# zihuixue/DynMM

Measured on AMD Instinct MI355X. Metric: images/sec fwd+bwd, 480x640 RGB-D, batch 32/GPU, higher is better.
Workload: dtype f32; 1 GPU; configs[2]: zero-grad + fwd + weighted 4-scale CE + FLOP loss + bwd + fused SGD-Nesterov update, --dynamic --global-gate soft DiffSoftmax gates tau=1; per_gpu_batch=32, global_batch=32, height=480, width=640, parallelism=dp1, launch=eager, streams=4, optimizer_in_step=fused SGD-Nesterov

## Files before the change

### dynmm_amd/csrc/conv_wino.hip

```cpp
#include <stdlib.h>

#include "common.h"
#include "conv_igemm.h"

namespace dynmm {

struct WinoArgs {
    const float* x;
    const float* ut;
    const float* shift;
    const float* residual;
    const float* mask;
    float* y;
    double* stats;
    const float *bn_mean, *bn_invstd, *bn_gamma, *bn_beta;
    const unsigned long long* bits;
    int nslots;
    int N, Ci, Co, H, W;
    int CoS;
    int act;
    int MP;
    int H2;
    int n_co_tiles, n_p_tiles;
    int Hin, Win;
};

__device__ __forceinline__ float quad_sum(float v) {
    v += __int_as_float(__builtin_amdgcn_mov_dpp(__float_as_int(v), 0xB1, 0xF, 0xF, true));
    v += __int_as_float(__builtin_amdgcn_mov_dpp(__float_as_int(v), 0x4E, 0xF, 0xF, true));
    return v;
}

template <int TCO, int MCO, bool VERT, bool DGRAD, bool S2 = false, bool TAIL = false, bool STATS = false, int BNRED = 0>
__global__ void __launch_bounds__(256, MCO == 1 ? ((VERT && !DGRAD) ? 4 : 3) : 2) conv_wino_kernel(const WinoArgs a) {
    static_assert(!BNRED || (DGRAD && VERT && !S2 && MCO == 1 && TCO == 64 && !TAIL && !STATS), "BatchNorm reductions: vertical dgrad");
    static_assert(!S2 || DGRAD, "the stride-2 form is an input gradient");
    static_assert(!STATS || (!DGRAD && !VERT && MCO == 1 && TCO == 64 && !TAIL), "statistics: the forward's small horizontal tile");
    static_assert(!TAIL || (!DGRAD && MCO == 1), "channel tails exist in the forward's small tile only");
    constexpr int S = (VERT && !DGRAD && MCO == 1) ? 2 : 3;
    constexpr int BK = 8;
    constexpr int WCO = 32 * MCO;
    constexpr int WAVES_CO = TCO / WCO, WAVES_P = 4 / WAVES_CO, TP = 32 * WAVES_P;
    static_assert(WAVES_CO * WAVES_P == 4 && (MCO == 1 || MCO == 2), "4 waves per workgroup");
    constexpr int A_STAGE = BK * TCO * 4;
    constexpr int PIXW = (S2 ? TP : 2 * TP) + 8;
    constexpr int NP = S2 ? 2 : 4;
    constexpr int B_STAGE = VERT ? BK * NP * TP : BK * PIXW;
    constexpr int QPR = VERT ? TP / 4 : PIXW / 4;
    constexpr int QB = B_STAGE / 4, QPW = QB / 4;
    constexpr int NIB = (QPW + 63) / 64;
    constexpr int IPR = TCO / 64;
    constexpr int NIA = 2 * IPR;
    constexpr int NI = NIA + NIB;
    static_assert(NI < 64 && QB % 4 == 0, "vmcnt is a 6-bit counter; the four waves split a stage evenly");

    __shared__ __attribute__((aligned(16))) float As[S * A_STAGE];
    __shared__ __attribute__((aligned(16))) float Bs[S * B_STAGE];

    const int t = threadIdx.x;
    const int lane = t & 63;
    const int wave = __builtin_amdgcn_readfirstlane(t >> 6);
    const int wave_co = wave / WAVES_P, wave_p = wave % WAVES_P;
    const int khalf = lane >> 5, l31 = lane & 31;

    const int nblk = a.n_co_tiles * a.n_p_tiles;
    const int lin = xcd_remap((int)blockIdx.x, nblk);
    const int co0 = (lin % a.n_co_tiles) * TCO;
    const int p0 = (lin / a.n_co_tiles) * TP;
    const int HW = a.H * a.W;
    const int HWin = a.Hin * a.Win;
    const int NC = a.Ci / BK;
    const int nst = NC;

    unsigned b_off[NIB];
    bool b_act[NIB];
#pragma unroll
    for (int i = 0; i < NIB; ++i) {
        const int ql = i * 64 + lane;
        b_act[i] = ql < QPW;
        const int q = wave * QPW + (b_act[i] ? ql : 0);
        if constexpr (VERT) {
            const int k = q / (NP * QPR), j = (q / QPR) % NP, gq = q % QPR;
            int p = p0 + 4 * gq;
            p = p > a.MP - 4 ? a.MP - 4 : p;
            const int per = a.H2 * a.W;
            const int n = p / per, rr = p - n * per;
            const int r2 = rr / a.W, w = rr - r2 * a.W;
            const int row = S2 ? r2 + j : 2 * r2 - 1 + j;
            const int rowc = (row >= 0 && row < a.Hin) ? row : (S2 ? r2 : 2 * r2);
            b_off[i] = ((unsigned)(n * a.Ci + k) * (unsigned)HWin + (unsigned)(rowc * a.Win + w)) * 4u;
        } else {
            const int k = q / QPR, quad = q - k * QPR;
            const int M = S2 ? a.MP : 2 * a.MP;
            int m = (S2 ? p0 : 2 * p0) - 4 + 4 * quad;
            m = m < 0 ? 0 : (m > M - 4 ? M - 4 : m);
            const int n = m / HWin, rem = m - n * HWin;
            b_off[i] = ((unsigned)(n * a.Ci + k) * (unsigned)HWin + (unsigned)rem) * 4u;
        }
    }
    const unsigned a_voff = (unsigned)lane * 16u;
    const unsigned lds_a = (unsigned)reinterpret_cast<uintptr_t>((__attribute__((address_space(3))) float*)As);
    const unsigned lds_b = (unsigned)reinterpret_cast<uintptr_t>((__attribute__((address_space(3))) float*)Bs);
    const float* a_ptr = a.ut + ((size_t)(2 * wave) * a.CoS + co0) * 4;
    const size_t a_step = (size_t)BK * a.CoS * 4, a_row = (size_t)a.CoS * 4;
    const float* b_ptr = a.x;
    const size_t b_step = (size_t)BK * HWin;
    unsigned l_adst = lds_a + (unsigned)(2 * wave * TCO * 4 * 4), l_bdst = lds_b + (unsigned)(wave * QPW * 4 * 4);
    const unsigned l_adst_end = l_adst + (unsigned)(S * A_STAGE * 4);
    int l_left = nst;
    auto issue = [&]() {
        if (l_left > 0) {
#pragma unroll
            for (int i = 0; i < NIA; ++i)
                dma16(a_ptr + (size_t)(i / IPR) * a_row + 64 * (i % IPR) * 4, a_voff, l_adst + (unsigned)i * 1024u);
#pragma unroll
            for (int i = 0; i < NIB; ++i) {
                if (b_act[i]) dma16(b_ptr, b_off[i], l_bdst + (unsigned)i * 1024u);
            }
            --l_left;
            a_ptr += a_step;
            b_ptr += b_step;
            l_adst += (unsigned)(A_STAGE * 4);
            l_bdst += (unsigned)(B_STAGE * 4);
            if (l_adst == l_adst_end) {
                l_adst -= (unsigned)(S * A_STAGE * 4);
                l_bdst -= (unsigned)(S * B_STAGE * 4);
            }
        }
    };

    const int lp = wave_p * 32 + l31;
    const int p = p0 + lp;
    const bool pvalid = p < a.MP;
    int pn, prem;
    bool m0, m2, m3;
    {
        const int pc = pvalid ? p : 0;
        if constexpr (VERT) {
            const int per = a.H2 * a.W;
            pn = pc / per;
            const int rr = pc - pn * per;
            const int r2 = rr / a.W, w = rr - r2 * a.W;
            prem = 2 * r2 * a.W + w;
            m0 = r2 > 0;
            m2 = 2 * r2 + 1 < a.H;
            m3 = S2 ? r2 + 1 < a.Hin : 2 * r2 + 2 < a.H;
        } else {
            const int m = 2 * pc;
            pn = m / HW;
            prem = m - pn * HW;
            const int h = prem / a.W, w = prem - h * a.W;
            m0 = w > 0;
            m2 = true;
            m3 = S2 ? (w >> 1) + 1 < a.Win : w + 2 < a.W;
        }
    }
    const int a_frag = (khalf * TCO + wave_co * WCO + l31) * 4;
    const int b_frag = VERT ? khalf * NP * TP + lp : (S2 ? khalf * PIXW + 4 + lp : khalf * PIXW + 2 * lp + 2);

    f32x16 acc[4][MCO];
#pragma unroll
    for (int i = 0; i < 4; ++i)
#pragma unroll
        for (int mi = 0; mi < MCO; ++mi)
#pragma unroll
            for (int j = 0; j < 16; ++j) acc[i][mi][j] = 0.f;

    float4 fa[2][MCO];
    float fd[2][4];
    float fv[2][4];
    auto read_raw = [&](int set, int q, const float* Ap, const float* Bp) {
#pragma unroll
        for (int mi = 0; mi < MCO; ++mi)
            fa[set][mi] = *reinterpret_cast<const float4*>(Ap + a_frag + (2 * q * TCO + mi * 32) * 4);
        if constexpr (S2) {
            const float* b = Bp + b_frag + 2 * q * (VERT ? NP * TP : PIXW);
            fd[set][0] = b[0];
            fd[set][1] = b[VERT ? TP : 1];
            fd[set][2] = fd[set][3] = 0.f;
        } else if constexpr (VERT) {
            const float* b = Bp + b_frag + 2 * q * 4 * TP;
            fd[set][0] = b[0];
            fd[set][1] = b[TP];
            fd[set][2] = b[2 * TP];
            fd[set][3] = b[3 * TP];
        } else {
            const float* b = Bp + b_frag + 2 * q * PIXW;
            const float2 u1 = *reinterpret_cast<const float2*>(b + 2);
            fd[set][0] = b[1];
            fd[set][1] = u1.x;
            fd[set][2] = u1.y;
            fd[set][3] = b[4];
        }
    };
    auto transform = [&](int set) {
        if constexpr (S2) {
            fv[set][0] = fv[set][1] = fd[set][0];
            fv[set][2] = m3 ? fd[set][1] : 0.f;
            fv[set][3] = 0.f;
            return;
        }
        const float d0 = m0 ? fd[set][0] : 0.f, d1 = fd[set][1];
        const float d2 = (VERT && !m2) ? 0.f : fd[set][2], d3 = m3 ? fd[set][3] : 0.f;
        fv[set][0] = d0 - d2;
        fv[set][1] = d1 + d2;
        fv[set][2] = d2 - d1;
        fv[set][3] = d1 - d3;
    };
    auto mfma_set = [&](int set) {
#pragma unroll
        for (int mi = 0; mi < MCO; ++mi) {
            const float av[4] = {fa[set][mi].x, fa[set][mi].y, fa[set][mi].z, fa[set][mi].w};
            if constexpr (S2) {
                acc[0][mi] = __builtin_amdgcn_mfma_f32_32x32x2f32(av[0], fv[set][0], acc[0][mi], 0, 0, 0);
                acc[1][mi] = __builtin_amdgcn_mfma_f32_32x32x2f32(av[1], fv[set][1], acc[1][mi], 0, 0, 0);
                acc[1][mi] = __builtin_amdgcn_mfma_f32_32x32x2f32(av[2], fv[set][2], acc[1][mi], 0, 0, 0);
                continue;
            }
#pragma unroll
            for (int i = 0; i < 4; ++i)
                acc[i][mi] = __builtin_amdgcn_mfma_f32_32x32x2f32(av[i], fv[set][i], acc[i][mi], 0, 0, 0);
        }
    };
#define DYNMM_WINO_PHASE() __builtin_amdgcn_sched_barrier(0)

    static_assert(BK == 8, "four k-pairs per stage");
#pragma unroll
    for (int i = 0; i < S; ++i) issue();
    wait_vm<(S - 1) * NI>();
    __syncthreads();
    int c_a = 0, c_b = 0;
    const float* Ap = As;
    const float* Bp = Bs;
    read_raw(0, 0, Ap, Bp);
    transform(0);
    for (int s = 0; s < nst; ++s) {
        DYNMM_WINO_PHASE();
        read_raw(1, 1, Ap, Bp);
        DYNMM_WINO_PHASE();
        mfma_set(0);
        DYNMM_WINO_PHASE();
        transform(1);
        DYNMM_WINO_PHASE();
        read_raw(0, 2, Ap, Bp);
        DYNMM_WINO_PHASE();
        mfma_set(1);
        DYNMM_WINO_PHASE();
        transform(0);
        DYNMM_WINO_PHASE();
        read_raw(1, 3, Ap, Bp);
        DYNMM_WINO_PHASE();
        mfma_set(0);
        DYNMM_WINO_PHASE();
        transform(1);
        DYNMM_WINO_PHASE();
        if (s + 1 < nst) {
            if (S > 2 && s + 2 < nst) wait_vm<(S - 2) * NI>();
            else wait_vm<0>();
            __syncthreads();
            issue();
            c_a += A_STAGE;
            c_b += B_STAGE;
            if (c_a == S * A_STAGE) { c_a = 0; c_b = 0; }
            Ap = As + c_a;
            Bp = Bs + c_b;
            read_raw(0, 0, Ap, Bp);
        }
        DYNMM_WINO_PHASE();
        mfma_set(1);
        DYNMM_WINO_PHASE();
        transform(0);
    }
#undef DYNMM_WINO_PHASE
    const float* __restrict__ res_p = a.residual;
    const float* __restrict__ mask_p = a.mask;
    float* __restrict__ y_p = a.y;
    const bool has_res = res_p != nullptr, has_mask = mask_p != nullptr;
    const int act = a.act;
    const unsigned row_bytes = (unsigned)HW * 4u;
    const unsigned second = VERT ? (unsigned)a.W * 4u : 4u;
    const bool y1_ok = VERT ? m2 : true;
    const unsigned off_base = ((unsigned)(pn * a.Co + co0 + wave_co * WCO + 4 * khalf) * (unsigned)HW + (unsigned)prem) * 4u;
    auto off_of = [&](int b, int e) {
        return off_base + (unsigned)((b >> 1) * 32 + (e & 3) + 8 * (2 * (b & 1) + (e >> 2))) * row_bytes;
    };
    const int co_lim = a.Co - (co0 + wave_co * WCO + 4 * khalf);
    auto live = [&](int b, int e) { return !TAIL || (b >> 1) * 32 + (e & 3) + 8 * (2 * (b & 1) + (e >> 2)) < co_lim; };
    constexpr int NSET = BNRED == 2 ? 1 : 2;
    float k0[NSET][8], k1[NSET][8], r0[NSET][8], r1[NSET][8];
    unsigned w0[NSET][8], w1[NSET][8];
    const unsigned bit_groups = (unsigned)((HW + 255) >> 8);
    auto bit_byte = [&](int i) { return (unsigned)(((i >> 8) * 4 + (i & 3)) * 8 + ((((i & 255) >> 2) >> 5) * 4)); };
    const unsigned bit_off0 = bit_byte(prem), bit_off1 = bit_byte(prem + a.W);
    const unsigned bit_sh0 = (unsigned)(((prem & 255) >> 2) & 31), bit_sh1 = (unsigned)((((prem + a.W) & 255) >> 2) & 31);
    const unsigned bit_plane0 = (unsigned)(pn * a.Co + co0 + wave_co * WCO + 4 * khalf) * bit_groups * 32u;
#pragma unroll
    for (int e = 0; e < 8; ++e)
#pragma unroll
        for (int q = 0; q < NSET; ++q) {
            r0[q][e] = r1[q][e] = 0.f;
            k0[q][e] = k1[q][e] = 1.f;
        }
    auto load_batch = [&](int set, int b) {
#pragma unroll
        for (int e = 0; e < 8; ++e) {
            const unsigned off = off_of(b, e);
            r0[set][e] = r1[set][e] = 0.f;
            k0[set][e] = k1[set][e] = 1.f;
            if constexpr (BNRED == 2) w0[set][e] = w1[set][e] = 0u;
            if (!pvalid || !live(b, e)) continue;
            if constexpr (BNRED == 2) {
                const char* wp_ = reinterpret_cast<const char*>(a.bits) + bit_plane0 +
                                  (unsigned)((b >> 1) * 32 + (e & 3) + 8 * (2 * (b & 1) + (e >> 2))) * bit_groups * 32u;
                w0[set][e] = *reinterpret_cast<const unsigned*>(wp_ + bit_off0);
                w1[set][e] = y1_ok ? *reinterpret_cast<const unsigned*>(wp_ + bit_off1) : 0u;
            }
            if constexpr (VERT) {
                if (has_mask) {
                    k0[set][e] = *reinterpret_cast<const float*>(reinterpret_cast<const char*>(mask_p) + off);
                    if (y1_ok) k1[set][e] = *reinterpret_cast<const float*>(reinterpret_cast<const char*>(mask_p) + off + second);
                }
                if (has_res) {
                    r0[set][e] = *reinterpret_cast<const float*>(reinterpret_cast<const char*>(res_p) + off);
                    if (y1_ok) r1[set][e] = *reinterpret_cast<const float*>(reinterpret_cast<const char*>(res_p) + off + second);
                }
            } else {
                if (has_mask) {
                    const float2 kk = *reinterpret_cast<const float2*>(reinterpret_cast<const char*>(mask_p) + off);
                    k0[set][e] = kk.x;
                    k1[set][e] = kk.y;
                }
                if (has_res) {
                    const float2 rr = *reinterpret_cast<const float2*>(reinterpret_cast<const char*>(res_p) + off);
                    r0[set][e] = rr.x;
                    r1[set][e] = rr.y;
                }
            }
        }
    };
    if (has_mask || has_res) load_batch(0, 0);
    __syncthreads();
    float* const sh_lds = As;
    for (int i = t; i < TCO; i += 256) sh_lds[i] = (a.shift && (!TAIL || co0 + i < a.Co)) ? a.shift[co0 + i] : 0.f;
    __syncthreads();
    float* const cst_lds = As + TCO;
    if constexpr (BNRED) {
        if (t < TCO) {
            const int c = co0 + t;
            const float is = a.bn_invstd[c], mu = a.bn_mean[c], sc = a.bn_gamma[c] * is;
            cst_lds[4 * t + 0] = sc;
            cst_lds[4 * t + 1] = fmaf(-mu, sc, a.bn_beta[c]);
            cst_lds[4 * t + 2] = is;
            cst_lds[4 * t + 3] = -mu * is;
        }
        __syncthreads();
    }
    if constexpr (!STATS && !BNRED) {
        if (!pvalid) return;
    }
    float* const st_lds = As + 5 * TCO;
#pragma unroll
    for (int b = 0; b < 2 * MCO; ++b) {
        const int mi = b >> 1, h = b & 1, set = NSET == 2 ? (b & 1) : 0;
        if constexpr (NSET == 2) {
            if (b + 1 < 2 * MCO && (has_mask || has_res)) load_batch(set ^ 1, b + 1);
        } else {
            if (b > 0) load_batch(0, b);
        }
        float v0[8], v1[8];
        float q1[8], q2[8];
#pragma unroll
        for (int e = 0; e < 8; ++e) {
            const int j = 8 * h + e;
            const float ma = acc[0][mi][j], mb = acc[1][mi][j], mc = acc[2][mi][j], md = acc[3][mi][j];
            const int cl = wave_co * WCO + mi * 32 + 4 * khalf + (e & 3) + 8 * (2 * h + (e >> 2));
            const float sh = sh_lds[cl];
            float y0 = S2 ? ma + sh : (ma + mb) + mc + sh;
            float y1 = S2 ? mb + sh : (mb - mc) - md + sh;
            if constexpr (BNRED != 0) {
                const float4 cs = *reinterpret_cast<const float4*>(cst_lds + 4 * cl);
                const float c0 = k0[set][e], c1 = k1[set][e];
                if constexpr (BNRED == 2) {
                    y0 = (pvalid && ((w0[set][e] >> bit_sh0) & 1u)) ? y0 + r0[set][e] : 0.f;
                    y1 = (pvalid && y1_ok && ((w1[set][e] >> bit_sh1) & 1u)) ? y1 + r1[set][e] : 0.f;
                } else {
                    y0 = (pvalid && fmaf(c0, cs.x, cs.y) > 0.f) ? y0 : 0.f;
                    y1 = (pvalid && y1_ok && fmaf(c1, cs.x, cs.y) > 0.f) ? y1 : 0.f;
                }
                q1[e] = y0 + y1;
                q2[e] = fmaf(y0, fmaf(c0, cs.z, cs.w), y1 * fmaf(c1, cs.z, cs.w));
            } else if (DGRAD) {
                if (has_mask) {
                    y0 = k0[set][e] > 0.f ? y0 : 0.f;
                    y1 = k1[set][e] > 0.f ? y1 : 0.f;
                }
                y0 += r0[set][e];
                y1 += r1[set][e];
            } else {
                y0 += r0[set][e];
                y1 += r1[set][e];
                if (act == DYNMM_ACT_RELU) {
                    y0 = y0 > 0.f ? y0 : 0.f;
                    y1 = y1 > 0.f ? y1 : 0.f;
                } else if (act == DYNMM_ACT_TANH) {
                    y0 = tanhf(y0);
                    y1 = tanhf(y1);
                } else if (act == DYNMM_ACT_SWISH) {
                    y0 = swish_fwd(y0);
                    y1 = swish_fwd(y1);
                } else if (act == DYNMM_ACT_HSWISH) {
                    y0 = hswish_fwd(y0);
                    y1 = hswish_fwd(y1);
                }
            }
            v0[e] = y0;
            v1[e] = y1;
        }
        if constexpr (STATS || BNRED) {
#pragma unroll
            for (int e = 0; e < 8; ++e) {
                const float s1 = quad_sum(BNRED ? q1[e] : (pvalid ? v0[e] + v1[e] : 0.f));
                const float s2 = quad_sum(BNRED ? q2[e] : (pvalid ? fmaf(v0[e], v0[e], v1[e] * v1[e]) : 0.f));
                if ((l31 & 3) == 0) {
                    float* dst = st_lds + ((b * 4 + wave) * 32 + (khalf * 8 + e) * 2) * 8 + (l31 >> 2);
                    dst[0] = s1;
                    dst[8] = s2;
                }
            }
        }
#pragma unroll
        for (int e = 0; e < 8; ++e) {
            const unsigned off = off_of(b, e);
            if (!live(b, e) || ((STATS || BNRED) && !pvalid)) continue;
            if constexpr (VERT) {
                *reinterpret_cast<float*>(reinterpret_cast<char*>(y_p) + off) = v0[e];
                if (y1_ok) *reinterpret_cast<float*>(reinterpret_cast<char*>(y_p) + off + second) = v1[e];
            } else {
                *reinterpret_cast<float2*>(reinterpret_cast<char*>(y_p) + off) = make_float2(v0[e], v1[e]);
            }
        }
        __builtin_amdgcn_sched_barrier(0);
    }
    if constexpr (STATS || BNRED) {
        __syncthreads();
        const int sb = t >> 7, r = (t >> 1) & 63, wp = t & 1;
        const int wco = r >> 5, row = r & 31;
        const float* src = st_lds + ((sb * 4 + wco * WAVES_P + wp) * 32 + row) * 8;
        float acc_s = 0.f;
#pragma unroll
        for (int j = 0; j < 8; ++j) acc_s += src[j];
        acc_s += __int_as_float(__builtin_amdgcn_mov_dpp(__float_as_int(acc_s), 0xB1, 0xF, 0xF, true));
        if (wp == 0) {
            const int kh = row >> 4, e = (row >> 1) & 7, stat = row & 1;
            const int c = co0 + wco * WCO + 4 * kh + (e & 3) + 8 * (2 * sb + (e >> 2));
            atomicAdd(a.stats + ((size_t)((lin / a.n_co_tiles) % a.nslots) * 2 + stat) * a.Co + c, (double)acc_s);
        }
    }
}

__global__ void __launch_bounds__(256) wino_pack_kernel(const float* __restrict__ w, float4* __restrict__ ut,
                                                        const float* __restrict__ scale, int Co, int Ci, int dgrad) {
    const int K = dgrad ? Co : Ci, Cr = dgrad ? Ci : Co, Cc = (Cr + 63) & ~63;
    const size_t total = (size_t)K * Cc;
    const size_t o = (size_t)blockIdx.x * 256 + threadIdx.x;
    if (o >= total) return;
    const int c = (int)(o % Cc);
    const int k = (int)(o / Cc);
    if (c >= Cr) {
        ut[o] = make_float4(0.f, 0.f, 0.f, 0.f);
        return;
    }
    const int co = dgrad ? k : c, ci = dgrad ? c : k;
    const float* g = w + ((size_t)co * Ci + ci) * 3;
    float g0 = g[0], g1 = g[1], g2 = g[2];
    if (dgrad == 2) {
        ut[o] = make_float4(g1, g2, g0, 0.f);
        return;
    }
    if (dgrad) { const float tmp = g0; g0 = g2; g2 = tmp; }
    if (scale) {
        const float sc = scale[co];
        g0 *= sc; g1 *= sc; g2 *= sc;
    }
    ut[o] = make_float4(g0, (g0 + g1 + g2) * 0.5f, (g0 - g1 + g2) * 0.5f, g2);
}

struct WinoPackDesc {
    long long src, dst;
    int Co, Ci, kk, blk0;
};

__global__ void __launch_bounds__(256) wino_pack_multi_kernel(const float* __restrict__ src_base, float* __restrict__ dst_base,
                                                              const WinoPackDesc* __restrict__ desc, int ndesc) {
    int lo = 0, hi = ndesc - 1;
    while (lo < hi) {
        const int mid = (lo + hi + 1) >> 1;
        if (desc[mid].blk0 <= (int)blockIdx.x) lo = mid;
        else hi = mid - 1;
    }
    const WinoPackDesc d = desc[lo];
    const int dgrad = (d.kk >> 16) & 3;
    const int K = dgrad ? d.Co : d.Ci, Cr = dgrad ? d.Ci : d.Co, Cc = (Cr + 63) & ~63;
    const size_t total = (size_t)K * Cc;
    const size_t o = (size_t)((int)blockIdx.x - d.blk0) * 256 + threadIdx.x;
    if (o >= total) return;
    const int c = (int)(o % Cc);
    const int k = (int)(o / Cc);
    if (c >= Cr) {
        reinterpret_cast<float4*>(dst_base + d.dst)[o] = make_float4(0.f, 0.f, 0.f, 0.f);
        return;
    }
    const int co = dgrad ? k : c, ci = dgrad ? c : k;
    const float* g = src_base + d.src + ((size_t)co * d.Ci + ci) * 3;
    float g0 = g[0], g1 = g[1], g2 = g[2];
    if (dgrad == 2) {
        reinterpret_cast<float4*>(dst_base + d.dst)[o] = make_float4(g1, g2, g0, 0.f);
        return;
    }
    if (dgrad) { const float tmp = g0; g0 = g2; g2 = tmp; }
    reinterpret_cast<float4*>(dst_base + d.dst)[o] = make_float4(g0, (g0 + g1 + g2) * 0.5f, (g0 - g1 + g2) * 0.5f, g2);
}

static bool wino_geom_ok(const dynmm_conv_geom* g, bool dgrad) {
    if (!g || g->c_split != g->Ci) return false;
    if (g->SH != 1 || g->SW != 1) return false;
    const bool k13 = g->KH == 1 && g->KW == 3, k31 = g->KH == 3 && g->KW == 1;
    if (!(k13 || k31)) return false;
    if (g->PH != g->KH / 2 || g->PW != g->KW / 2 || g->H != g->Ho || g->W != g->Wo) return false;
    if (g->W % 4 != 0 || g->W < 4 || g->H < 2) return false;
    const int rows = dgrad ? g->Ci : g->Co, red = dgrad ? g->Co : g->Ci;
    if ((dgrad ? rows % 64 != 0 : (rows % 8 != 0 || rows < 24)) || red % 8 != 0 || red < 24) return false;
    if ((long long)g->N * g->H * g->W < 256) return false;
    if ((double)g->N * (g->Ci > g->Co ? g->Ci : g->Co) * g->H * g->W >= 1073741824.0) return false;
    return true;
}

static bool wino_s2_geom_ok(const dynmm_conv_geom* g) {
    if (!g || g->c_split != g->Ci) return false;
    const bool v = g->KH == 3 && g->KW == 1 && g->SH == 2 && g->SW == 1 && g->PH == 1 && g->PW == 0;
    const bool h = g->KH == 1 && g->KW == 3 && g->SH == 1 && g->SW == 2 && g->PH == 0 && g->PW == 1;
    if (!v && !h) return false;
    if (v && (g->H % 2 != 0 || g->Ho * 2 != g->H || g->Wo != g->W)) return false;
    if (h && (g->W % 2 != 0 || g->Wo * 2 != g->W || g->Ho != g->H)) return false;
    if (g->W % 4 != 0 || g->Wo % 4 != 0 || g->Wo < 4 || g->Ho < 1) return false;
    if (g->Ci % 64 != 0 || g->Co % 8 != 0 || g->Co < 24) return false;
    if ((long long)g->N * g->Ho * g->Wo < 256) return false;
    if ((double)g->N * (g->Ci > g->Co ? g->Ci : g->Co) * g->H * g->W >= 1073741824.0) return false;
    return true;
}

static int launch_wino(WinoArgs& a, bool vert, bool dgrad, hipStream_t st, bool s2 = false) {
    if (s2) {
        a.H2 = a.Hin;
        a.MP = a.N * a.Hin * a.Win;
        a.n_co_tiles = a.Co / 64;
        a.n_p_tiles = ceil_div(a.MP, 64);
        dim3 grid2((unsigned)(a.n_co_tiles * a.n_p_tiles));
        if (vert) hipLaunchKernelGGL((conv_wino_kernel<64, 1, true, true, true>), grid2, dim3(256), 0, st, a);
        else hipLaunchKernelGGL((conv_wino_kernel<64, 1, false, true, true>), grid2, dim3(256), 0, st, a);
        DYNMM_LAUNCH_CHECK();
        return DYNMM_OK;
    }
    a.Hin = a.H;
    a.Win = a.W;
    a.H2 = (a.H + 1) / 2;
    a.MP = vert ? a.N * a.H2 * a.W : a.N * a.H * a.W / 2;
    const bool tail = a.Co % 64 != 0;
    a.n_co_tiles = ceil_div(a.Co, 64);
    a.n_p_tiles = ceil_div(a.MP, 64);
    dim3 grid((unsigned)(a.n_co_tiles * a.n_p_tiles));
#define DYNMM_WINO_LAUNCH(...) hipLaunchKernelGGL((conv_wino_kernel<64, 1, __VA_ARGS__>), grid, dim3(256), 0, st, a)
    if (a.stats && dgrad) {
        if (a.bits) DYNMM_WINO_LAUNCH(true, true, false, false, false, 2);
        else DYNMM_WINO_LAUNCH(true, true, false, false, false, 1);
    } else if (a.stats) {
        DYNMM_WINO_LAUNCH(false, false, false, false, true);
    } else if (tail) {
        if (vert) DYNMM_WINO_LAUNCH(true, false, false, true);
        else DYNMM_WINO_LAUNCH(false, false, false, true);
    } else if (vert) {
        if (dgrad) DYNMM_WINO_LAUNCH(true, true);
        else DYNMM_WINO_LAUNCH(true, false);
    } else {
        if (dgrad) DYNMM_WINO_LAUNCH(false, true);
        else DYNMM_WINO_LAUNCH(false, false);
    }
#undef DYNMM_WINO_LAUNCH
    DYNMM_LAUNCH_CHECK();
    return DYNMM_OK;
}

}

using namespace dynmm;

extern "C" int dynmm_conv2d_wino_supported(const dynmm_conv_geom* g, int dgrad) {
    if (wino_geom_ok(g, dgrad != 0)) return 1;
    return (dgrad && wino_s2_geom_ok(g)) ? 2 : 0;
}

extern "C" size_t dynmm_wino_packed_floats(int Co, int Ci, int KH, int KW) {
    if (Co <= 0 || Ci <= 0 || KH <= 0 || KW <= 0) return 0;
    if (!((KH == 1 && KW == 3) || (KH == 3 && KW == 1))) return 0;
    const size_t fwd = (size_t)Ci * ((Co + 63) & ~63), dg = (size_t)Co * ((Ci + 63) & ~63);
    return (fwd > dg ? fwd : dg) * 4;
}

extern "C" int dynmm_wino_pack(const float* w, float* ut, const float* scale, int Co, int Ci, int KH, int KW, int dgrad,
                               void* stream) {
    (void)hipGetLastError();
    if (!w || !ut || Co <= 0 || Ci <= 0 || (scale && dgrad) || dgrad < 0 || dgrad > 2) return DYNMM_EINVAL;
    if (!((KH == 1 && KW == 3) || (KH == 3 && KW == 1))) return DYNMM_EUNSUPPORTED;
    if (reinterpret_cast<uintptr_t>(ut) & 15u) return DYNMM_EINVAL;
    const size_t total = dynmm_wino_packed_floats(Co, Ci, KH, KW) / 4;
    hipLaunchKernelGGL(wino_pack_kernel, dim3((unsigned)ceil_div_sz(total, 256)), dim3(256), 0, (hipStream_t)stream, w,
                       reinterpret_cast<float4*>(ut), scale, Co, Ci, dgrad);
    DYNMM_LAUNCH_CHECK();
    return DYNMM_OK;
}

extern "C" int dynmm_wino_pack_multi_blocks(int Co, int Ci, int KH, int KW) {
    return (int)ceil_div_sz(dynmm_wino_packed_floats(Co, Ci, KH, KW) / 4, 256);
}

extern "C" int dynmm_wino_pack_multi(const float* src_base, float* dst_base, const void* desc, int ndesc, int total_blocks,
                                     void* stream) {
    (void)hipGetLastError();
    if (!src_base || !dst_base || !desc || ndesc <= 0 || total_blocks <= 0) return DYNMM_EINVAL;
    if (reinterpret_cast<uintptr_t>(dst_base) & 15u) return DYNMM_EINVAL;
    static_assert(sizeof(WinoPackDesc) == 32, "descriptor layout is part of the ABI (4 x int64 words)");
    hipLaunchKernelGGL(wino_pack_multi_kernel, dim3(total_blocks), dim3(256), 0, (hipStream_t)stream, src_base, dst_base,
                       (const WinoPackDesc*)desc, ndesc);
    DYNMM_LAUNCH_CHECK();
    return DYNMM_OK;
}

extern "C" int dynmm_conv2d_wino_fwd(const float* x, const float* ut, const float* bias, const float* residual, float* y,
                                     const dynmm_conv_geom* g, int act, void* stream) {
    (void)hipGetLastError();
    if (!x || !ut || !y || !g) return DYNMM_EINVAL;
    if (!act_is_known(act)) return DYNMM_EINVAL;
    if (!wino_geom_ok(g, false)) return DYNMM_EUNSUPPORTED;
    if ((reinterpret_cast<uintptr_t>(x) | reinterpret_cast<uintptr_t>(ut)) & 15u) return DYNMM_EUNSUPPORTED;
    if ((reinterpret_cast<uintptr_t>(y) | reinterpret_cast<uintptr_t>(residual)) & 7u) return DYNMM_EUNSUPPORTED;
    WinoArgs a{};
    a.x = x; a.ut = ut; a.shift = bias; a.residual = residual; a.mask = nullptr; a.y = y;
    a.N = g->N; a.Ci = g->Ci; a.Co = g->Co; a.H = g->H; a.W = g->W;
    a.CoS = (g->Co + 63) & ~63;
    a.act = act;
    return launch_wino(a, g->KW == 1, false, (hipStream_t)stream);
}

extern "C" int dynmm_conv2d_wino_dgrad_bnred_supported(const dynmm_conv_geom* g) {
    return (wino_geom_ok(g, true) && g->KH == 3 && g->KW == 1 && g->Ci % 64 == 0) ? 1 : 0;
}

extern "C" int dynmm_conv2d_wino_dgrad_bnred_slots(const dynmm_conv_geom* g) {
    if (!dynmm_conv2d_wino_dgrad_bnred_supported(g)) return 0;
    const int s = ceil_div(g->N * ((g->H + 1) / 2) * g->W, 64) / 600;
    return s < 1 ? 1 : (s > 8 ? 8 : s);
}

extern "C" int dynmm_conv2d_wino_dgrad_bnred(const float* dy, const float* ut, const float* bn_x, const float* bn_mean,
                                             const float* bn_invstd, const float* bn_gamma, const float* bn_beta,
                                             double* sums, float* dx, const dynmm_conv_geom* g, void* stream) {
    (void)hipGetLastError();
    if (!dy || !ut || !bn_x || !bn_mean || !bn_invstd || !bn_gamma || !bn_beta || !sums || !dx || !g) return DYNMM_EINVAL;
    if (!dynmm_conv2d_wino_dgrad_bnred_supported(g)) return DYNMM_EUNSUPPORTED;
    if ((reinterpret_cast<uintptr_t>(dy) | reinterpret_cast<uintptr_t>(ut)) & 15u) return DYNMM_EUNSUPPORTED;
    if ((reinterpret_cast<uintptr_t>(dx) | reinterpret_cast<uintptr_t>(bn_x) | reinterpret_cast<uintptr_t>(sums)) & 7u)
        return DYNMM_EUNSUPPORTED;
    WinoArgs a{};
    a.x = dy; a.ut = ut; a.shift = nullptr; a.residual = nullptr; a.mask = bn_x; a.y = dx;
    a.stats = sums; a.nslots = dynmm_conv2d_wino_dgrad_bnred_slots(g);
    a.bn_mean = bn_mean; a.bn_invstd = bn_invstd; a.bn_gamma = bn_gamma; a.bn_beta = bn_beta;
    a.N = g->N; a.Ci = g->Co; a.Co = g->Ci; a.H = g->H; a.W = g->W;
    a.CoS = (a.Co + 63) & ~63;
    a.act = DYNMM_ACT_NONE;
    a.Hin = g->Ho; a.Win = g->Wo;
    return launch_wino(a, true, true, (hipStream_t)stream);
}

extern "C" int dynmm_conv2d_wino_dgrad_bnred2(const float* dy, const float* ut, const float* accum, const float* bn_x,
                                              const unsigned long long* relu_bits, const float* bn_mean, const float* bn_invstd,
                                              double* sums, float* dx, const dynmm_conv_geom* g, void* stream) {
    (void)hipGetLastError();
    if (!dy || !ut || !bn_x || !relu_bits || !bn_mean || !bn_invstd || !sums || !dx || !g) return DYNMM_EINVAL;
    if (!dynmm_conv2d_wino_dgrad_bnred_supported(g) || (g->H * g->W) % 4 != 0) return DYNMM_EUNSUPPORTED;
    if ((reinterpret_cast<uintptr_t>(dy) | reinterpret_cast<uintptr_t>(ut)) & 15u) return DYNMM_EUNSUPPORTED;
    if ((reinterpret_cast<uintptr_t>(dx) | reinterpret_cast<uintptr_t>(bn_x) | reinterpret_cast<uintptr_t>(accum) |
         reinterpret_cast<uintptr_t>(sums) | reinterpret_cast<uintptr_t>(relu_bits)) & 7u)
        return DYNMM_EUNSUPPORTED;
    WinoArgs a{};
    a.x = dy; a.ut = ut; a.shift = nullptr; a.residual = accum; a.mask = bn_x; a.y = dx;
    a.stats = sums; a.nslots = dynmm_conv2d_wino_dgrad_bnred_slots(g); a.bits = relu_bits;
    a.bn_mean = bn_mean; a.bn_invstd = bn_invstd; a.bn_gamma = bn_invstd; a.bn_beta = bn_invstd;
    a.N = g->N; a.Ci = g->Co; a.Co = g->Ci; a.H = g->H; a.W = g->W;
    a.CoS = (a.Co + 63) & ~63;
    a.act = DYNMM_ACT_NONE;
    a.Hin = g->Ho; a.Win = g->Wo;
    return launch_wino(a, true, true, (hipStream_t)stream);
}

extern "C" int dynmm_conv2d_wino_fwd_stats_supported(const dynmm_conv_geom* g) {
    return (wino_geom_ok(g, false) && g->KW == 3 && g->Co % 64 == 0) ? 1 : 0;
}

extern "C" int dynmm_conv2d_wino_fwd_stats_slots(const dynmm_conv_geom* g) {
    if (!dynmm_conv2d_wino_fwd_stats_supported(g)) return 0;
    const int tiles = ceil_div(g->N * g->H * g->W / 2, 64);
    const int s = tiles / 600;
    return s < 1 ? 1 : (s > 8 ? 8 : s);
}

extern "C" int dynmm_conv2d_wino_fwd_stats(const float* x, const float* ut, const float* bias, float* y, double* stats,
                                           int nslots, const dynmm_conv_geom* g, void* stream) {
    (void)hipGetLastError();
    if (!x || !ut || !y || !stats || !g || nslots < 1 || nslots > 64) return DYNMM_EINVAL;
    if (!dynmm_conv2d_wino_fwd_stats_supported(g)) return DYNMM_EUNSUPPORTED;
    if ((reinterpret_cast<uintptr_t>(x) | reinterpret_cast<uintptr_t>(ut)) & 15u) return DYNMM_EUNSUPPORTED;
    if ((reinterpret_cast<uintptr_t>(y) | reinterpret_cast<uintptr_t>(stats)) & 7u) return DYNMM_EUNSUPPORTED;
    WinoArgs a{};
    a.x = x; a.ut = ut; a.shift = bias; a.residual = nullptr; a.mask = nullptr; a.y = y; a.stats = stats; a.nslots = nslots;
    a.N = g->N; a.Ci = g->Ci; a.Co = g->Co; a.H = g->H; a.W = g->W;
    a.CoS = g->Co;
    a.act = DYNMM_ACT_NONE;
    return launch_wino(a, false, false, (hipStream_t)stream);
}

extern "C" int dynmm_conv2d_wino_dgrad(const float* dy, const float* ut, const float* mask, const float* accum, float* dx,
                                       const dynmm_conv_geom* g, void* stream) {
    (void)hipGetLastError();
    if (!dy || !ut || !dx || !g) return DYNMM_EINVAL;
    const bool s2 = !wino_geom_ok(g, true) && wino_s2_geom_ok(g);
    if (!s2 && !wino_geom_ok(g, true)) return DYNMM_EUNSUPPORTED;
    if ((reinterpret_cast<uintptr_t>(dy) | reinterpret_cast<uintptr_t>(ut)) & 15u) return DYNMM_EUNSUPPORTED;
    if ((reinterpret_cast<uintptr_t>(dx) | reinterpret_cast<uintptr_t>(mask) | reinterpret_cast<uintptr_t>(accum)) & 7u)
        return DYNMM_EUNSUPPORTED;
    WinoArgs a{};
    a.x = dy; a.ut = ut; a.shift = nullptr; a.residual = accum; a.mask = mask; a.y = dx;
    a.N = g->N; a.Ci = g->Co; a.Co = g->Ci; a.H = g->H; a.W = g->W;
    a.CoS = (a.Co + 63) & ~63;
    a.act = DYNMM_ACT_NONE;
    a.Hin = g->Ho; a.Win = g->Wo;
    return launch_wino(a, g->KW == 1, true, (hipStream_t)stream, s2);
}
```

Baseline: 511.4 images/s.

## Run vertical Winograd dgrad at four workgroups with half-batch epilogue loads

For the vertical input-gradient Winograd kernel, the launch bound is raised to four workgroups per CU and the staging ring is shrunk from three stages to two, so more workgroups can be resident at once. To fit the tighter register budget, the epilogue first folds the Winograd outputs into per-thread arrays, then walks the data in half-batches of four elements. Mask, residual and bit loads for the next half-batch are double-buffered behind the current one. This trades pipeline depth and epilogue register pressure for occupancy, with a risk of spills or weaker latency hiding in the main loop.

```diff
diff --git a/dynmm_amd/csrc/conv_wino.hip b/dynmm_amd/csrc/conv_wino.hip
--- a/dynmm_amd/csrc/conv_wino.hip
+++ b/dynmm_amd/csrc/conv_wino.hip
@@ -31,13 +31,29 @@
     return v;
 }
 
+#ifndef DYNMM_WINO_VDGRAD_WG4_PLAIN
+#define DYNMM_WINO_VDGRAD_WG4_PLAIN 1
+#endif
+#ifndef DYNMM_WINO_VDGRAD_WG4_BN1
+#define DYNMM_WINO_VDGRAD_WG4_BN1 1
+#endif
+#ifndef DYNMM_WINO_VDGRAD_WG4_BN2
+#define DYNMM_WINO_VDGRAD_WG4_BN2 1
+#endif
+constexpr bool wino_four_workgroups(int MCO, bool VERT, bool DGRAD, bool S2, int BNRED) {
+    if (MCO != 1 || !VERT || S2) return false;
+    if (!DGRAD) return true;
+    return BNRED == 0 ? DYNMM_WINO_VDGRAD_WG4_PLAIN : (BNRED == 1 ? DYNMM_WINO_VDGRAD_WG4_BN1 : DYNMM_WINO_VDGRAD_WG4_BN2);
+}
+
 template <int TCO, int MCO, bool VERT, bool DGRAD, bool S2 = false, bool TAIL = false, bool STATS = false, int BNRED = 0>
-__global__ void __launch_bounds__(256, MCO == 1 ? ((VERT && !DGRAD) ? 4 : 3) : 2) conv_wino_kernel(const WinoArgs a) {
+__global__ void __launch_bounds__(256, MCO == 1 ? (wino_four_workgroups(MCO, VERT, DGRAD, S2, BNRED) ? 4 : 3) : 2)
+conv_wino_kernel(const WinoArgs a) {
     static_assert(!BNRED || (DGRAD && VERT && !S2 && MCO == 1 && TCO == 64 && !TAIL && !STATS), "BatchNorm reductions: vertical dgrad");
     static_assert(!S2 || DGRAD, "the stride-2 form is an input gradient");
     static_assert(!STATS || (!DGRAD && !VERT && MCO == 1 && TCO == 64 && !TAIL), "statistics: the forward's small horizontal tile");
     static_assert(!TAIL || (!DGRAD && MCO == 1), "channel tails exist in the forward's small tile only");
-    constexpr int S = (VERT && !DGRAD && MCO == 1) ? 2 : 3;
+    constexpr int S = wino_four_workgroups(MCO, VERT, DGRAD, S2, BNRED) ? 2 : 3;
     constexpr int BK = 8;
     constexpr int WCO = 32 * MCO;
     constexpr int WAVES_CO = TCO / WCO, WAVES_P = 4 / WAVES_CO, TP = 32 * WAVES_P;
@@ -338,7 +354,48 @@
             }
         }
     };
-    if (has_mask || has_res) load_batch(0, 0);
+    constexpr bool HALF = VERT && DGRAD && !S2 && MCO == 1 && !TAIL && !STATS;
+    float hk0[2][4], hk1[2][4], hr0[2][4], hr1[2][4];
+    unsigned hw0[2][4], hw1[2][4];
+    const unsigned off_base1 = off_base + (y1_ok ? second : 0u);
+    const unsigned bit_base0 = bit_plane0 + bit_off0, bit_base1 = bit_plane0 + (y1_ok ? bit_off1 : bit_off0);
+    const unsigned long long* __restrict__ bits_p = a.bits;
+    auto ld32 = [](const void* base, unsigned off) { return *reinterpret_cast<const unsigned*>(reinterpret_cast<const char*>(base) + off); };
+    auto load_sub = [&](int set, int sb) {
+        const bool ld_mask = BNRED ? true : has_mask;
+        const bool ld_res = BNRED == 2 ? true : (BNRED == 1 ? false : has_res);
+        const float* res_src = (BNRED == 2 && !has_res) ? mask_p : res_p;
+        const int b = sb >> 1;
+#pragma unroll
+        for (int e4 = 0; e4 < 4; ++e4) {
+            const int e = 4 * (sb & 1) + e4;
+            const unsigned ch = (unsigned)((b >> 1) * 32 + (e & 3) + 8 * (2 * (b & 1) + (e >> 2)));
+            if constexpr (BNRED == 2) {
+                hw0[set][e4] = ld32(bits_p, bit_base0 + ch * (bit_groups * 32u));
+                hw1[set][e4] = ld32(bits_p, bit_base1 + ch * (bit_groups * 32u));
+            }
+            if (ld_mask) {
+                hk0[set][e4] = __uint_as_float(ld32(mask_p, off_base + ch * row_bytes));
+                hk1[set][e4] = __uint_as_float(ld32(mask_p, off_base1 + ch * row_bytes));
+            }
+            if (ld_res) {
+                hr0[set][e4] = __uint_as_float(ld32(res_src, off_base + ch * row_bytes));
+                hr1[set][e4] = __uint_as_float(ld32(res_src, off_base1 + ch * row_bytes));
+            }
+        }
+    };
+    if constexpr (HALF) {
+#pragma unroll
+        for (int e4 = 0; e4 < 4; ++e4)
+#pragma unroll
+            for (int q = 0; q < 2; ++q) {
+                hr0[q][e4] = hr1[q][e4] = 0.f;
+                hk0[q][e4] = hk1[q][e4] = 1.f;
+            }
+        if (BNRED || has_mask || has_res) load_sub(0, 0);
+    } else {
+        if (has_mask || has_res) load_batch(0, 0);
+    }
     __syncthreads();
     float* const sh_lds = As;
     for (int i = t; i < TCO; i += 256) sh_lds[i] = (a.shift && (!TAIL || co0 + i < a.Co)) ? a.shift[co0 + i] : 0.f;
@@ -359,6 +416,79 @@
         if (!pvalid) return;
     }
     float* const st_lds = As + 5 * TCO;
+    static_assert(5 * TCO + 2 * 4 * 32 * 8 <= S * A_STAGE, "the reduction scratch lies inside the filter ring");
+    if constexpr (HALF) {
+        float ty0[MCO][16], ty1[MCO][16];
+#pragma unroll
+        for (int mi = 0; mi < MCO; ++mi)
+#pragma unroll
+            for (int j = 0; j < 16; ++j) {
+                const int h = j >> 3, e = j & 7;
+                const float ma = acc[0][mi][j], mb = acc[1][mi][j], mc = acc[2][mi][j], md = acc[3][mi][j];
+                const float sh = sh_lds[wave_co * WCO + mi * 32 + 4 * khalf + (e & 3) + 8 * (2 * h + (e >> 2))];
+                ty0[mi][j] = (ma + mb) + mc + sh;
+                ty1[mi][j] = (mb - mc) - md + sh;
+                asm volatile("" : "+v"(ty0[mi][j]), "+v"(ty1[mi][j]));
+            }
+        __builtin_amdgcn_sched_barrier(0);
+#pragma unroll
+        for (int sb = 0; sb < 4 * MCO; ++sb) {
+            const int b = sb >> 1, mi = b >> 1, h = b & 1, set = sb & 1;
+            if (sb + 1 < 4 * MCO && (BNRED || has_mask || has_res)) load_sub(set ^ 1, sb + 1);
+            float v0[4], v1[4];
+            float q1[4], q2[4];
+#pragma unroll
+            for (int e4 = 0; e4 < 4; ++e4) {
+                const int e = 4 * (sb & 1) + e4, j = 8 * h + e;
+                const int cl = wave_co * WCO + mi * 32 + 4 * khalf + (e & 3) + 8 * (2 * h + (e >> 2));
+                float y0 = ty0[mi][j], y1 = ty1[mi][j];
+                if constexpr (BNRED != 0) {
+                    const float4 cs = *reinterpret_cast<const float4*>(cst_lds + 4 * cl);
+                    const float c0 = pvalid ? hk0[set][e4] : 1.f, c1 = (pvalid && y1_ok) ? hk1[set][e4] : 1.f;
+                    if constexpr (BNRED == 2) {
+                        const float a0 = has_res ? hr0[set][e4] : 0.f, a1 = has_res ? hr1[set][e4] : 0.f;
+                        y0 = (pvalid && ((hw0[set][e4] >> bit_sh0) & 1u)) ? y0 + a0 : 0.f;
+                        y1 = (pvalid && y1_ok && ((hw1[set][e4] >> bit_sh1) & 1u)) ? y1 + a1 : 0.f;
+                    } else {
+                        y0 = (pvalid && fmaf(c0, cs.x, cs.y) > 0.f) ? y0 : 0.f;
+                        y1 = (pvalid && y1_ok && fmaf(c1, cs.x, cs.y) > 0.f) ? y1 : 0.f;
+                    }
+                    q1[e4] = y0 + y1;
+                    q2[e4] = fmaf(y0, fmaf(c0, cs.z, cs.w), y1 * fmaf(c1, cs.z, cs.w));
+                } else {
+                    if (has_mask) {
+                        y0 = hk0[set][e4] > 0.f ? y0 : 0.f;
+                        y1 = hk1[set][e4] > 0.f ? y1 : 0.f;
+                    }
+                    y0 += hr0[set][e4];
+                    y1 += hr1[set][e4];
+                }
+                v0[e4] = y0;
+                v1[e4] = y1;
+            }
+            if constexpr (BNRED != 0) {
+#pragma unroll
+                for (int e4 = 0; e4 < 4; ++e4) {
+                    const int e = 4 * (sb & 1) + e4;
+                    const float s1 = quad_sum(q1[e4]);
+                    const float s2 = quad_sum(q2[e4]);
+                    if ((l31 & 3) == 0) {
+                        float* dst = st_lds + ((b * 4 + wave) * 32 + (khalf * 8 + e) * 2) * 8 + (l31 >> 2);
+                        dst[0] = s1;
+                        dst[8] = s2;
+                    }
+                }
+            }
+#pragma unroll
+            for (int e4 = 0; e4 < 4; ++e4) {
+                const unsigned off = off_of(b, 4 * (sb & 1) + e4);
+                if (BNRED && !pvalid) continue;
+                *reinterpret_cast<float*>(reinterpret_cast<char*>(y_p) + off) = v0[e4];
+                if (y1_ok) *reinterpret_cast<float*>(reinterpret_cast<char*>(y_p) + (off + second)) = v1[e4];
+            }
+            __builtin_amdgcn_sched_barrier(0);
+        }
+    } else {
 #pragma unroll
     for (int b = 0; b < 2 * MCO; ++b) {
         const int mi = b >> 1, h = b & 1, set = NSET == 2 ? (b & 1) : 0;
@@ -440,6 +570,7 @@
             }
         }
         __builtin_amdgcn_sched_barrier(0);
+    }
     }
     if constexpr (STATS || BNRED) {
         __syncthreads();
```

Result: no change. 514.3 images/s, median of 3 (+0.6%).
